# eridgd/WCT-TF

Hardware: AMD Instinct MI355X
Metric: stylized frames/sec @512x512, 5-level relu5->1 pipeline, alpha=0.8 (higher is better)
Workload: dtype f16

## Files before the change

wct_tf_amd/csrc/common.h:

```cpp
#pragma once
#include <hip/hip_runtime.h>
#include <stdint.h>
#include <stddef.h>
#include "skip_rule.h"

typedef _Float16 half_t;
typedef _Float16 half8 __attribute__((ext_vector_type(8)));
typedef _Float16 half4 __attribute__((ext_vector_type(4)));
typedef float f32x16 __attribute__((ext_vector_type(16)));
typedef float f32x4 __attribute__((ext_vector_type(4)));

#define WCT_OK 0
#define WCT_ERR_HIP -1
#define WCT_ERR_ARG -2
#define WCT_ERR_STATE -3
#define WCT_ERR_NOMEM -4
#define WCT_ERR_NOCONV -5

void wct_set_error(const char* fmt, ...);

#define HIP_TRY(expr)                                                          \
  do {                                                                         \
    hipError_t _e = (expr);                                                    \
    if (_e != hipSuccess) {                                                    \
      wct_set_error("%s failed: %s (%s:%d)", #expr, hipGetErrorString(_e),     \
                    __FILE__, __LINE__);                                       \
      return WCT_ERR_HIP;                                                      \
    }                                                                          \
  } while (0)

#define ARG_CHECK(cond)                                                        \
  do {                                                                         \
    if (!(cond)) {                                                             \
      wct_set_error("invalid argument: %s (%s:%d)", #cond, __FILE__, __LINE__);\
      return WCT_ERR_ARG;                                                      \
    }                                                                          \
  } while (0)

static inline int cdiv(int a, int b) { return (a + b - 1) / b; }

constexpr size_t WCT_LAUNCH_BYTES = (size_t)1 << 31;
static inline bool launch_map_fits(size_t elems, size_t bytes) { return elems * bytes < WCT_LAUNCH_BYTES; }


struct ConvArgs {
  const half_t* x;
  const half_t* w;
  const float* bias;
  half_t* y16;
  float* y32;
  int B, H, W;
  int Cin, Cout;
  int upsample;
  int relu;
  int pool;
  float* usum;
  unsigned* umax;
  const float* img1 = nullptr;
  const half_t* w1frag = nullptr;
  const float* bias1 = nullptr;
  int clamp01 = 0;
  const half_t* w_wino = nullptr;
};
constexpr int UMAX_SLOTS = 64;
__device__ __forceinline__ void umax_merge(unsigned* umax_img, int slot, float vmax, int lane) {
#pragma unroll
  for (int o = 32; o > 0; o >>= 1) vmax = fmaxf(vmax, __shfl_xor(vmax, o, 64));
  if (lane == 0) {
    unsigned* w = umax_img + (slot & (UMAX_SLOTS - 1));
    const unsigned bits = __builtin_bit_cast(unsigned, vmax);
    if (bits > __atomic_load_n(w, __ATOMIC_RELAXED)) atomicMax(w, bits);
  }
}
int launch_conv3x3(const ConvArgs& a, hipStream_t s);
bool conv3x3_wino_takes(const ConvArgs& a);
int launch_conv3x3_wino(const ConvArgs& a, hipStream_t s);

struct ConvFirstArgs {
  const float* x;
  const half_t* wfrag;
  const float* bias;
  half_t* y16;
  float* y32;
  int B, H, W;
  int clamp01;
  float* usum;
  unsigned* umax;
};

__device__ __forceinline__ void unit_row_sum4(f32x4& t) {
  float a = t[0], b = t[1], c = t[2], d = t[3];
#define WCT_DPP_STEP(ctrl)                                                             \
  "v_add_f32_dpp %0, %0, %0 " ctrl " row_mask:0xf bank_mask:0xf bound_ctrl:1\n"       \
  "v_add_f32_dpp %1, %1, %1 " ctrl " row_mask:0xf bank_mask:0xf bound_ctrl:1\n"       \
  "v_add_f32_dpp %2, %2, %2 " ctrl " row_mask:0xf bank_mask:0xf bound_ctrl:1\n"       \
  "v_add_f32_dpp %3, %3, %3 " ctrl " row_mask:0xf bank_mask:0xf bound_ctrl:1\n"
  asm volatile("s_nop 1\n"
               WCT_DPP_STEP("quad_perm:[1,0,3,2]")
               WCT_DPP_STEP("quad_perm:[2,3,0,1]")
               WCT_DPP_STEP("row_half_mirror")
               WCT_DPP_STEP("row_mirror")
               : "+v"(a), "+v"(b), "+v"(c), "+v"(d));
#undef WCT_DPP_STEP
  t[0] = a; t[1] = b; t[2] = c; t[3] = d;
}
int launch_conv_first(const ConvFirstArgs& a, hipStream_t s);

struct ConvLastArgs {
  const half_t* x;
  const half_t* wfrag;
  const float* bias;
  float* y;
  int B, H, W;
};
int launch_conv_last(const ConvLastArgs& a, hipStream_t s);

int launch_maxpool2x2(const half_t* x, half_t* y, int B, int H, int W, int C, hipStream_t s);
int launch_u8_to_f32(const uint8_t* x, float* y, size_t n, hipStream_t s);
int launch_f32_to_u8(const float* x, uint8_t* y, size_t n, hipStream_t s);
int launch_f32_to_f16(const float* x, half_t* y, size_t n, hipStream_t s);
int launch_f16_to_f32(const half_t* x, float* y, size_t n, hipStream_t s);

struct GemmArgs {
  const float* A; int lda; int a_kmajor;
  const float* B; int ldb; int b_kmajor;
  const float* a_sub_m;
  const float* b_sub_n;
  const float* a_sub_k;
  const float* a_scale_k;
  int M, N, K;
  int ksplit;
  float* out32; half_t* out16; int ldo;
  size_t out_split_stride;
  const float* bias_n;
  int nsplit;
  size_t sA, sB, s_sub_m, s_sub_n, s_sub_k, s_scale_k, s_out, s_bias;
  const float* A_odd;
  size_t sA_odd;
  WctSkip skip;
  int blend; float alpha; unsigned* mabs;
  const float* mask_diag; size_t s_mask; int* mask_out; const int* mask_in;
};

int launch_gemm(GemmArgs g, int nsplit, int nbatch, hipStream_t s);

enum { WCT_MODE_NP = 0, WCT_MODE_TF = 1 };

struct WctFeatStats { const float* u[2]; const unsigned* umax[2]; };

struct WctImageSide { const float* img; int H, W, clamp01; };
struct WctImageSrc { WctImageSide side[2]; const half_t* wfrag; const float* bias; };

struct WctStyleKey { int nslab, nsplit, ksplit; };
WctStyleKey wct_style_key(int C, int Nc, int Ns);
size_t wct_style_state_floats(int C);
size_t wct_style_workspace_bytes(int C, int Ns, const WctStyleKey& key);
struct WctStyleRef { const float* state[8]; };
struct WctStyleSlots { const float* state[32]; };

struct WctWarmRef { float* basis; int valid; };

struct WctStrength { const uint8_t* smap; int Hm, Wm, w, stride; };

struct WctCall {
  float alpha; int mode;
  float eps;
  half_t* out16; float* out32;
  void* workspace; size_t workspace_bytes;
  int* sweeps_dev;
  int stages;
  int* eig_fail;
  hipStream_t stream;
};
enum { WCT_STAGE_COV = 1, WCT_STAGE_EIG = 2, WCT_STAGE_APPLY = 4, WCT_STAGE_ALL = 7, WCT_STAGE_EIG_FP32UPDATE = 8 };

int launch_style_state(const float* style, int Ns, int C, const WctStyleKey& key, int adain, const WctCall& r, float* state);

size_t wct_workspace_bytes(int C, int Nc, int Ns, int P);
int launch_wct(const float* content, int Nc, const float* style, int Ns, int C, int P, WctSkip skip, const WctCall& r,
               const WctFeatStats* stats, const WctStyleRef* prep, const WctWarmRef* warm, const WctStrength* sm = nullptr,
               const WctImageSrc* src = nullptr );
int launch_adain(const float* content, int Nc, const float* style, int Ns, int C, int P, WctSkip skip, const WctCall& r,
                 const WctFeatStats* stats, const WctStyleRef* prep, const WctStrength* sm = nullptr);
enum { WCT_MIX_MAX = 8 };
size_t wct_mix_workspace_bytes(int C, int Nc, const int* Ns, int K, const float* lambda);
int launch_wct_mix(const float* content, int Nc, const float* const* styles, const int* Ns, int K, const float* lambda, int C,
                   const WctCall& r, const WctFeatStats* stats, const WctStyleRef* prep);
int launch_adain_mix(const float* content, int Nc, const float* const* styles, const int* Ns, int K, const float* lambda, int C,
                     const WctCall& r, const WctFeatStats* stats, const WctStyleRef* prep);
struct MaskGeom { const uint8_t* mask; int Hm, Wm, w, stride; };
size_t mask_compact_workspace_bytes(int N, int G = 1);
int launch_mask_compact(const MaskGeom& g, int N, int K, int* perm, int* seg_off, void* workspace, hipStream_t s);
int launch_mask_gather_segment(const float* x, const int* perm, const int* seg_off, int k, int nk, int C, float* xg, hipStream_t s);
size_t wct_masked_workspace_bytes(int C, int Nc, const int* nk, const int* Ns, int K);
int launch_wct_masked(const float* content, int Nc, const MaskGeom& g, const int* nk, const float* const* styles, const int* Ns, int K,
                      int C, const WctCall& r);
int launch_adain_masked(const float* content, int Nc, const MaskGeom& g, const int* nk, const float* const* styles, const int* Ns, int K,
                        int C, const WctCall& r);
size_t wct_masked_batch_workspace_bytes(int C, int Nc, int G, const int* nk, const int* Ns, int K);
int wct_masked_batch_pairs(int G, const int* nk, int K);
int launch_mask_compact_batch(const MaskGeom& g, int N, int K, int G, int* perm, int* seg_off, void* workspace, hipStream_t s);
int launch_wct_masked_batch(const float* content, int Nc, int G, const MaskGeom& g, const int* nk, const int* Ns, int K, int C,
                            const WctCall& r, const WctStyleSlots& states);
int launch_adain_masked_batch(const float* content, int Nc, int G, const MaskGeom& g, const int* nk, const int* Ns, int K, int C,
                              const WctCall& r, const WctStyleSlots& states);
int launch_jacobi_eigh(float* A, float* V, int C, int nmat, void* workspace,
                       size_t workspace_bytes, int* sweeps_done_dev, int* eig_fail, hipStream_t s);
size_t jacobi_workspace_bytes(int C, int nmat);

size_t style_swap_workspace_bytes(int C, int hc, int wc, int hs, int ws, int patch, int stride);
int launch_style_swap(const float* content, int hc, int wc, const float* style, int hs, int ws, int C,
                      float alpha, int patch, int stride, float eps, half_t* out16, float* out32,
                      void* workspace, size_t workspace_bytes, hipStream_t s, int* eig_fail);

int launch_im2col_act(const half_t* x, float* col, int B, int H, int W, int C, int upsample, hipStream_t s);
int launch_im2col_grad(const float* g, float* col, int B, int H, int W, int C, hipStream_t s);
int launch_reflect_fold(const float* gp, float* g, int B, int H, int W, int C, hipStream_t s);
int launch_relu_mask16(float* g, const half_t* act, size_t n, hipStream_t s);
int launch_relu_mask32(float* g, const float* act, size_t n, hipStream_t s);
int launch_upsample_adjoint(const float* gb, float* gs, int B, int h, int w, int C, hipStream_t s);
int launch_maxpool_adjoint(const half_t* pre, const float* gpool, float* gpre, int B, int H, int W, int C, hipStream_t s);
int launch_mse(const float* a, const float* b, size_t n, float weight, float* grad, int accumulate, double* partial,
               float* loss_out, hipStream_t s);
int launch_tv(const float* x, int B, int H, int W, int C, float weight, float* grad, double* partial, float* loss_out, hipStream_t s);
int launch_bias_grad(const float* g, size_t rows, int C, float* partial, float* out, hipStream_t s);
int launch_reduce_slabs(const float* partial, size_t n, int nslab, float* out, hipStream_t s);
int launch_adam(float* w, float* m, float* v, const float* g, size_t n, float lr_t, float b1, float b2, float eps, hipStream_t s);
int launch_pack_conv_frag(const float* w, half_t* frag, int cin, int cout, hipStream_t s);
int launch_pack_conv_wino_frag(const float* w, half_t* frag, int cin, int cout, hipStream_t s);
int launch_pack_last_frag(const float* w, half_t* frag, hipStream_t s);
int launch_transpose_w(const float* w, float* wt, int cin, int cout, int cout_pad, hipStream_t s);
int launch_pad3to4(const float* x, float* y, size_t n, hipStream_t s);
int launch_conv_dgrad(const float* g, const float* wt, int B, int H, int W, int cin, int cout,
                      float* col, float* gp, float* gin, void* scratch, hipStream_t s);
int launch_conv_wgrad(const half_t* x16, int upsample, const float* g, int ldg, int B, int H, int W, int cin, int cout,
                      float* col, float* partial, int nsplit, float* dw, void* scratch, hipStream_t s);
int conv_wgrad_splits(int B, int H, int W);
int launch_pow2_scale(const float* x, size_t n, void* scratch, hipStream_t s);
int launch_conv_first_dgrad(const float* g, const float* wf, float* gp, int B, int H, int W, hipStream_t s);

struct CoralApplyArgs {
  double M[9], src_mean[3], src_std[3], tgt_mean[3], tgt_std[3];
};
int launch_coral_stats(const uint8_t* img, size_t npix, unsigned long long* partial, int nblocks,
                       unsigned long long* out9, hipStream_t s);
int launch_coral_apply(const uint8_t* src, size_t npix, const CoralApplyArgs& a, uint8_t* out_u8,
                       double* out_f64, hipStream_t s);

int launch_content_colors_f32(const float* frame, const void* content, int content_f32, int B, int Ho, int Wo, int Hc, int Wc,
                              uint8_t* out, hipStream_t s);
int launch_content_colors_u8(const uint8_t* stylized, const uint8_t* content, int B, int Ho, int Wo, int Hc, int Wc, uint8_t* out,
                             hipStream_t s);
int launch_content_colors_u8_any(const uint8_t* stylized, const void* content, int content_f32, int B, int Ho, int Wo, int Hc, int Wc,
                                 uint8_t* out, hipStream_t s);

constexpr int GUIDE_GREY = 0, GUIDE_COLOR = 1;
int guided_check(int B, int Ho, int Wo, int Hc, int Wc, int radius, int eps_q, int guide);
size_t guided_workspace_bytes(int B, int Ho, int Wo, int guide);
int launch_guided_filter(const uint8_t* stylized, const void* content, int content_f32, int B, int Ho, int Wo, int Hc, int Wc, int radius,
                         int eps_q, int guide, void* workspace, uint8_t* out, hipStream_t s);
int launch_guided_color(const uint8_t* stylized, const void* content, int content_f32, int B, int Ho, int Wo, int Hc, int Wc, int radius,
                        int eps_q, void* workspace, uint8_t* out, hipStream_t s);
int guided_time_check(int F, int Ho, int Wo, int Hc, int Wc, int radius, int eps_q, int frames_t, int f0, int f1);
int guided_time_max_radius(int frames_t);
int launch_guided_time(const uint8_t* stylized, const void* content, int content_f32, int F, int Ho, int Wo, int Hc, int Wc, int radius,
                       int eps_q, int frames_t, int f0, int f1, void* workspace, uint8_t* out, hipStream_t s);
int guided_motion_check(int F, int Ho, int Wo, int Hc, int Wc, int radius, int eps_q, int frames_t, int f0, int f1, const int32_t* pos);
int launch_guided_motion(const uint8_t* stylized, const uint8_t* content, int F, int Ho, int Wo, int Hc, int Wc, int radius, int eps_q,
                         int frames_t, const int32_t* pos, int f0, int f1, void* workspace, uint8_t* out, hipStream_t s);
int motion_check(int F, int Hc, int Wc, int range);
size_t motion_workspace_bytes(int F, int Hc, int Wc, int range);
int launch_motion_global(const uint8_t* content, int F, int Hc, int Wc, int range, void* workspace, const int32_t** steps, hipStream_t s);

int launch_texture_noise(uint8_t* out, int B, int H, int W, unsigned seed, unsigned first_sample, int smooth, hipStream_t s);

int launch_wrap_pad(const void* in, void* out, int B, int H, int W, int E, int elem_bytes, int t, int b, int l, int r, hipStream_t s);
int launch_wrap_crop(const void* in, void* out, int B, int Hp, int Wp, int E, int elem_bytes, int t, int l, int h, int w, hipStream_t s);

struct ResizeGeom { int H, W, h, w, ksx, ksy, th; };
int resize_check_bytes(int B, int H, int W, int h, int w);
size_t resize_table_ints(int H, int W, int h, int w);
int resize_plan(int H, int W, int h, int w, ResizeGeom* g, int* tabs);
int launch_resize(const uint8_t* in, uint8_t* out, int B, const ResizeGeom& g, const int* tabs_dev, hipStream_t s);
```

wct_tf_amd/csrc/spectral.hip:

```cpp
#include "wct_stages.h"

__device__ __forceinline__ bool pair_resolved(float dp, float dq, float e) { return e * e <= 0.25f * dp * dq; }

constexpr float SPECTRAL_NOISE_CUT = 2.f;
__device__ __forceinline__ float spectral_cut(const float* Am, int C, int tid, float* red) {
  float mn = 0.f;
  for (int i = tid; i < C; i += 256) mn = fminf(mn, Am[(size_t)i * C + i]);
  for (int o = 32; o > 0; o >>= 1) mn = fminf(mn, __shfl_xor(mn, o, 64));
  if ((tid & 63) == 0) red[tid >> 6] = mn;
  __syncthreads();
  mn = fminf(fminf(red[0], red[1]), fminf(red[2], red[3]));
  return fmaxf(1e-5f, -SPECTRAL_NOISE_CUT * mn);
}

__device__ __forceinline__ float spectral_entry(float dp, float dq, float e, bool diag, int kind, float shift, float cut) {
  const bool kp = dp > cut, kq = dq > cut;
  if (diag) return kp ? (kind == 0 ? 1.f / sqrtf(dp + shift) : sqrtf(dp + shift)) : 0.f;
  if (!kp && !kq) return 0.f;
  if (kp && kq) {
    if (!pair_resolved(dp, dq, e)) return 0.f;
    const float sa = sqrtf(dp + shift), sb = sqrtf(dq + shift);
    return kind == 0 ? -e / (sa * sb * (sa + sb)) : e / (sa + sb);
  }
  const float dk = kp ? dp : dq, dd = kp ? dq : dp;
  const float fk = kind == 0 ? 1.f / sqrtf(dk + shift) : sqrtf(dk + shift);
  return e * fk / fmaxf(dk - dd, 2.f * fabsf(e));
}

struct SpectralTile {
  float dp[64], dq[64];
  float mt[64][65];
};
__attribute__((used)) __device__ __forceinline__ void spectral_tile_load(SpectralTile& t, const float* Am, int C, int p0, int q0, int tid) {
  if (tid < 64) t.dp[tid] = p0 + tid < C ? Am[(size_t)(p0 + tid) * C + p0 + tid] : 0.f;
  else if (tid < 128) t.dq[tid - 64] = q0 + tid - 64 < C ? Am[(size_t)(q0 + tid - 64) * C + q0 + tid - 64] : 0.f;
  const int ty = tid >> 4, tx = tid & 15;
#pragma unroll
  for (int i = 0; i < 4; ++i) {
    const int r = q0 + ty * 4 + i, c = p0 + tx * 4;
    f32x4 v = {0.f, 0.f, 0.f, 0.f};
    if (r < C && c < C) v = *reinterpret_cast<const f32x4*>(Am + (size_t)r * C + c);
#pragma unroll
    for (int j = 0; j < 4; ++j) t.mt[ty * 4 + i][tx * 4 + j] = v[j];
  }
}

struct SpecAllArgs {
  const float* A;
  float* G;
  float *N, *R, *Pm;
  const float *X1, *X2;
  int C; float shift; int correct, second; WctSkip skip;
  unsigned* mabs; const float* mean; float* bias; float alpha; int mode;
};

__global__ __launch_bounds__(256) void spectral_open_all_kernel(SpecAllArgs a) {
  __shared__ SpectralTile t;
  const int m = blockIdx.z, p0 = blockIdx.y * 64, q0 = blockIdx.x * 64, tid = threadIdx.x;
  const int C = a.C, kind = m & 1, pair = m >> 1;
  const size_t cc = (size_t)C * C;
  if (kind == 0 && blockIdx.x == 0 && blockIdx.y == 0) {
    if (tid == 0) a.mabs[pair] = 0u;
    const float* mp = a.mean + (size_t)(one_content(a.skip) ? 0 : pair) * 2 * C;
    const float* ms = a.mean + (size_t)(one_style(a.skip) ? 0 : pair) * 2 * C + C;
    for (int i = tid; i < C; i += 256) {
      float b = a.alpha * ms[i];
      if (a.mode == WCT_MODE_TF) b += (1.f - a.alpha) * mp[i];
      a.bias[pair * C + i] = b;
    }
  }
  if (skip_style_mat(m, a.skip)) return;
  __shared__ float cutred[4];
  const float* Am = a.A + m * cc;
  const float cut = spectral_cut(Am, C, tid, cutred);
  spectral_tile_load(t, Am, C, p0, q0, tid);
  __syncthreads();
  const int ty = tid >> 4, tx = tid & 15;
#pragma unroll
  for (int i = 0; i < 4; ++i) {
    const int pl = ty * 4 + i, p = p0 + pl, q = q0 + tx * 4;
    if (p >= C || q >= C) continue;
    const f32x4 av = *reinterpret_cast<const f32x4*>(Am + (size_t)p * C + q);
    const float dp = t.dp[pl];
    f32x4 g, n4 = {0.f, 0.f, 0.f, 0.f}, r4 = n4, p4 = n4;
#pragma unroll
    for (int j = 0; j < 4; ++j) {
      const float dk = t.dq[tx * 4 + j];
      const float em = 0.5f * (av[j] + t.mt[tx * 4 + j][pl]);
      g[j] = spectral_entry(dp, dk, a.correct ? em : 0.f, p == q + j, kind, a.shift, cut);
      if (a.second && p != q + j && dp > cut && dk > cut && pair_resolved(dp, dk, em)) {
        const float sp = sqrtf(dp + a.shift), sk = sqrtf(dk + a.shift);
        n4[j] = em / (sp + sk);
        r4[j] = em / sk;
        p4[j] = n4[j] / sk;
      }
    }
    const size_t o = (size_t)p * C + q;
    *reinterpret_cast<f32x4*>(a.G + m * cc + o) = g;
    if (a.second) {
      *reinterpret_cast<f32x4*>(a.N + m * cc + o) = n4;
      if (kind == 0) { *reinterpret_cast<f32x4*>(a.R + pair * cc + o) = r4; *reinterpret_cast<f32x4*>(a.Pm + pair * cc + o) = p4; }
    }
  }
}

__global__ __launch_bounds__(256) void spectral_add2_all_kernel(SpecAllArgs a) {
  __shared__ float dps[64], dqs[64];
  __shared__ float x1t[64][65], x2t[64][65];
  const int m = blockIdx.z, p0 = blockIdx.y * 64, q0 = blockIdx.x * 64, tid = threadIdx.x;
  if (skip_style_mat(m, a.skip)) return;
  const int C = a.C, kind = m & 1;
  const size_t cc = (size_t)C * C;
  const float* Am = a.A + m * cc;
  float* Gm = a.G + m * cc;
  const float* X2 = a.X2 + m * cc;
  const float* X1 = a.X1 + (size_t)(m >> 1) * cc;
  int near = 0;
  for (int i = tid; i < C; i += 256) {
    const float d = fabsf(Am[(size_t)i * C + i]);
    near |= (d > 3.3e-6f) & (d < 3e-5f);
  }
  if (__syncthreads_or(near)) return;
  __shared__ float cutred[4];
  const float cut = spectral_cut(Am, C, tid, cutred);
  if (tid < 64) dps[tid] = p0 + tid < C ? Am[(size_t)(p0 + tid) * C + p0 + tid] : 0.f;
  else if (tid < 128) dqs[tid - 64] = q0 + tid - 64 < C ? Am[(size_t)(q0 + tid - 64) * C + q0 + tid - 64] : 0.f;
  const int ty = tid >> 4, tx = tid & 15;
#pragma unroll
  for (int i = 0; i < 4; ++i) {
    const int r = q0 + ty * 4 + i, c = p0 + tx * 4;
    f32x4 v1 = {0.f, 0.f, 0.f, 0.f}, v2 = v1;
    if (r < C && c < C) {
      v2 = *reinterpret_cast<const f32x4*>(X2 + (size_t)r * C + c);
      if (kind == 0) v1 = *reinterpret_cast<const f32x4*>(X1 + (size_t)r * C + c);
    }
#pragma unroll
    for (int j = 0; j < 4; ++j) { x2t[ty * 4 + i][tx * 4 + j] = v2[j]; x1t[ty * 4 + i][tx * 4 + j] = v1[j]; }
  }
  __syncthreads();
#pragma unroll
  for (int i = 0; i < 4; ++i) {
    const int pl = ty * 4 + i, p = p0 + pl, q = q0 + tx * 4;
    if (p >= C || q >= C) continue;
    const size_t o = (size_t)p * C + q;
    const f32x4 x2 = *reinterpret_cast<const f32x4*>(X2 + o);
    f32x4 x1 = {0.f, 0.f, 0.f, 0.f};
    if (kind == 0) x1 = *reinterpret_cast<const f32x4*>(X1 + o);
    f32x4 g = *reinterpret_cast<const f32x4*>(Gm + o);
    const float dp = dps[pl];
#pragma unroll
    for (int j = 0; j < 4; ++j) {
      const float dq = dqs[tx * 4 + j];
      if (!(dp > cut && dq > cut)) continue;
      const float sp = sqrtf(dp + a.shift), sq = sqrtf(dq + a.shift);
      float l2;
      if (kind == 1) l2 = -0.5f * (x2[j] + x2t[tx * 4 + j][pl]) / (sp + sq);
      else l2 = (0.5f * (x1[j] + x1t[tx * 4 + j][pl]) + 0.25f * (sp + sq) * (x2[j] + x2t[tx * 4 + j][pl])) / (sp * sq * (sp + sq));
      g[j] += l2;
    }
    *reinterpret_cast<f32x4*>(Gm + o) = g;
  }
}

static GemmArgs level_product(int C, WctSkip skip) {
  GemmArgs g = {};
  g.lda = g.ldb = g.ldo = C; g.M = g.N = g.K = g.ksplit = C; g.sA = g.sB = g.s_out = (size_t)C * C; g.skip = skip;
  return g;
}

static int launch_refresh(const WctCarve& w, int C, int P, WctSkip skip, hipStream_t s) {
  int rc;
  GemmArgs r1 = level_product(C, skip);
  r1.A = w.A0; r1.a_kmajor = 0; r1.B = w.V; r1.b_kmajor = 1; r1.out32 = w.X;
  r1.mask_diag = w.A; r1.s_mask = (size_t)C * C; r1.mask_out = w.refresh;
  if ((rc = launch_gemm(r1, 1, 2 * P, s))) return rc;
  GemmArgs r2 = level_product(C, skip);
  r2.A = w.V; r2.a_kmajor = 1; r2.B = w.X; r2.b_kmajor = 1; r2.out32 = w.A; r2.mask_in = w.refresh;
  return launch_gemm(r2, 1, 2 * P, s);
}

int launch_spectral_tail_refreshed(const WctCarve& w, int C, int P, float alpha, int mode, float eps_in, WctSkip skip, int nwhite,
                                   hipStream_t s) {
  int rc;
  const size_t cc = (size_t)C * C;
  const float shift = mode == WCT_MODE_NP ? (eps_in >= 0.f ? eps_in : 1e-5f) : 0.f;
  const int second = EIG_CORRECT >= 2;
  const dim3 tiles(cdiv(C, 64), cdiv(C, 64), 2 * P);
  SpecAllArgs sa = {};
  sa.A = w.A; sa.G = w.G; sa.C = C; sa.shift = shift; sa.correct = EIG_CORRECT; sa.second = second; sa.skip = skip;
  sa.N = w.S2; float* X2 = sa.N + 2 * P * cc; sa.R = X2 + 2 * P * cc; sa.Pm = sa.R + P * cc; float* X1 = sa.Pm + P * cc;
  sa.X1 = X1; sa.X2 = X2;
  sa.mabs = w.mabs; sa.mean = w.mean; sa.bias = w.bias; sa.alpha = alpha; sa.mode = mode;
  hipLaunchKernelGGL(spectral_open_all_kernel, tiles, dim3(256), 0, s, sa);
  HIP_TRY(hipGetLastError());
  if (second) {
    GemmArgs a = level_product(C, skip);
    a.A = sa.Pm; a.A_odd = sa.N + cc; a.sA_odd = 2 * cc; a.a_kmajor = 0; a.B = sa.N; a.b_kmajor = 1; a.out32 = X2;
    if ((rc = launch_gemm(a, 1, 2 * P, s))) return rc;
    GemmArgs b = level_product(C, WCT_SKIP_NONE);
    b.A = sa.R; b.a_kmajor = 0; b.B = sa.N; b.b_kmajor = 1; b.sB = 2 * cc; b.out32 = X1;
    if (nwhite > 0 && (rc = launch_gemm(b, 1, nwhite, s))) return rc;
    hipLaunchKernelGGL(spectral_add2_all_kernel, tiles, dim3(256), 0, s, sa);
    HIP_TRY(hipGetLastError());
  }
  GemmArgs g = level_product(C, skip);
  g.A = w.V; g.a_kmajor = 0; g.B = w.G; g.b_kmajor = 1; g.out32 = w.X;
  if ((rc = launch_gemm(g, 1, 2 * P, s))) return rc;
  GemmArgs h = level_product(C, skip);
  h.A = w.X; h.a_kmajor = 0; h.B = w.V; h.b_kmajor = 0; h.out32 = w.Tw;
  return launch_gemm(h, 1, 2 * P, s);
}

int launch_spectral_tail(const WctCarve& w, int C, int P, float alpha, int mode, float eps_in, WctSkip skip, int nwhite,
                         hipStream_t s) {
  const int rc = launch_refresh(w, C, P, skip, s);
  return rc ? rc : launch_spectral_tail_refreshed(w, C, P, alpha, mode, eps_in, skip, nwhite, s);
}
```

wct_tf_amd/csrc/stats_gemm.hip:

```cpp
#include "wct_stages.h"
#include "conv_first_tile.h"
#include <type_traits>


struct StatArgs {
  const float* x[2];
  int n[2];
  const float* u[2];
  const unsigned* umax[2];
  const float* mean;
  float* partial;
  float* absmax;
  int C, nslab;
  WctSkip skip;
};

__global__ __launch_bounds__(256) void colsum_kernel(StatArgs p) {
  __shared__ f32x4 red[256];
  const int mat = blockIdx.y, slab = blockIdx.x;
  if (skip_style_mat(mat, p.skip)) return;
  const int b = mat & 1, pair = mat >> 1;
  const int C = p.C, cq = C / 4;
  const int nrp = 256 / cq;
  const int tid = threadIdx.x;
  const int rp = tid / cq, c4 = tid % cq;
  const int N = p.n[b];
  const float* x = p.x[b] + (size_t)pair * N * C;
  f32x4 acc = {0.f, 0.f, 0.f, 0.f};
  float amax = 0.f;
  if (p.mean) {
    const int rows_per_slab = (N + p.nslab - 1) / p.nslab;
    const int r0 = slab * rows_per_slab;
    const int r1 = min(N, r0 + rows_per_slab);
    const f32x4 m = *reinterpret_cast<const f32x4*>(p.mean + mat * C + c4 * 4);
    if (rp < nrp)
      for (int r = r0 + rp; r < r1; r += nrp) {
        f32x4 v = *reinterpret_cast<const f32x4*>(x + (size_t)r * C + c4 * 4);
        v -= m; acc += v * v;
      }
  } else {
    const int units = (N + 15) >> 4;
    const int ups = (units + p.nslab - 1) / p.nslab;
    const int u0 = slab * ups, u1 = min(units, u0 + ups);
    const float* U = p.u[b] ? p.u[b] + (size_t)pair * units * C : nullptr;
    if (rp < nrp)
      for (int u = u0 + rp; u < u1; u += nrp) {
        if (U) {
          acc += *reinterpret_cast<const f32x4*>(U + (size_t)u * C + c4 * 4);
        } else {
          f32x4 t[16];
#pragma unroll
          for (int i = 0; i < 16; ++i) {
            const int r = u * 16 + i;
            t[i] = *reinterpret_cast<const f32x4*>(x + (size_t)min(r, N - 1) * C + c4 * 4);
            if (r >= N) t[i] = f32x4{0.f, 0.f, 0.f, 0.f};
            amax = fmaxf(fmaxf(amax, fmaxf(fabsf(t[i][0]), fabsf(t[i][1]))), fmaxf(fabsf(t[i][2]), fabsf(t[i][3])));
          }
#pragma unroll
          for (int w = 1; w < 16; w <<= 1)
#pragma unroll
            for (int i = 0; i < 16; i += 2 * w) t[i] += t[i + w];
          acc += t[0];
        }
      }
    if (U) amax = __builtin_bit_cast(float, p.umax[b][pair * UMAX_SLOTS + (tid & (UMAX_SLOTS - 1))]);
  }
  red[tid] = acc;
  __syncthreads();
  if (rp == 0) {
    for (int j = 1; j < nrp; ++j) acc += red[j * cq + c4];
    *reinterpret_cast<f32x4*>(p.partial + ((size_t)mat * p.nslab + slab) * C + c4 * 4) = acc;
  }
  if (p.absmax) {
    __syncthreads();
    float* redf = reinterpret_cast<float*>(red);
    redf[tid] = amax;
    __syncthreads();
    for (int st = 128; st > 0; st >>= 1) {
      if (tid < st) redf[tid] = fmaxf(redf[tid], redf[tid + st]);
      __syncthreads();
    }
    if (tid == 0) p.absmax[(size_t)mat * p.nslab + slab] = redf[0];
  }
}

__global__ void colsum_finish_kernel(const float* partial, float* out, int C, int nslab, float d0, float d1, int skip,
                                     const float* absmax = nullptr, float* scale = nullptr) {
  const int mat = blockIdx.y;
  if (skip_style_mat(mat, skip)) return;
  if (scale && blockIdx.x == 0 && threadIdx.x < 64) {
    float m = 0.f;
    for (int i = threadIdx.x; i < nslab; i += 64) m = fmaxf(m, absmax[(size_t)mat * nslab + i]);
    for (int o = 32; o > 0; o >>= 1) m = fmaxf(m, __shfl_xor(m, o, 64));
    if (threadIdx.x == 0) {
      float sc = 1.f;
      if (m > 0.f && m < 1e30f) {
        int e;
        frexpf(2.f * m, &e);
        sc = ldexpf(1.f, 14 - e);
      }
      scale[mat] = sc;
    }
  }
  const int c = blockIdx.x * blockDim.x + threadIdx.x;
  if (c >= C) return;
  float a[8] = {0.f, 0.f, 0.f, 0.f, 0.f, 0.f, 0.f, 0.f};
  const float* pp = partial + (size_t)mat * nslab * C + c;
  int i = 0;
  for (; i + 8 <= nslab; i += 8) {
#pragma unroll
    for (int j = 0; j < 8; ++j) a[j] += pp[(size_t)(i + j) * C];
  }
  for (; i < nslab; ++i) a[i & 7] += pp[(size_t)i * C];
  const float s = ((a[0] + a[1]) + (a[2] + a[3])) + ((a[4] + a[5]) + (a[6] + a[7]));
  out[mat * C + c] = s / ((mat & 1) == 0 ? d0 : d1);
}

constexpr int GK = 16;

template <int BX>
struct GemmStage {
  static constexpr int NV = GK * BX / 4 / 256;
  f32x4 v[NV];
  __device__ __forceinline__ void load(const float* src, int ld, bool kmajor, int k0, int kend, int x0, int X,
                                       const float* sub_x, const float* sub_k, const float* scale_k, int tid) {
#pragma unroll
    for (int i = 0; i < NV; ++i) {
      const int item = tid + i * 256;
      f32x4 t = {0.f, 0.f, 0.f, 0.f};
      if (kmajor) {
        const int k = item / (BX / 4), x4 = item % (BX / 4);
        const int gk = k0 + k, gx = x0 + x4 * 4;
        if (gk < kend && gx < X) {
          t = *reinterpret_cast<const f32x4*>(src + (size_t)gk * ld + gx);
          if (sub_x) t -= *reinterpret_cast<const f32x4*>(sub_x + gx);
        }
      } else {
        const int x = item / (GK / 4), k4 = item % (GK / 4);
        const int gx = x0 + x, gk = k0 + k4 * 4;
        if (gx < X && gk < kend) {
          t = *reinterpret_cast<const f32x4*>(src + (size_t)gx * ld + gk);
          if (sub_k) t -= *reinterpret_cast<const f32x4*>(sub_k + gk);
          if (scale_k) t *= *reinterpret_cast<const f32x4*>(scale_k + gk);
        }
      }
      v[i] = t;
    }
  }
  __device__ __forceinline__ void store(float* lds , bool kmajor, int tid) const {
    constexpr int P = BX + 4;
#pragma unroll
    for (int i = 0; i < NV; ++i) {
      const int item = tid + i * 256;
      if (kmajor) {
        const int k = item / (BX / 4), x4 = item % (BX / 4);
        *reinterpret_cast<f32x4*>(lds + k * P + x4 * 4) = v[i];
      } else {
        const int x = item / (GK / 4), k4 = item % (GK / 4);
#pragma unroll
        for (int j = 0; j < 4; ++j) lds[(k4 * 4 + j) * P + x] = v[i][j];
      }
    }
  }
};

constexpr float REFRESH_RATIO = 1e-4f;
__device__ __forceinline__ bool refresh_needed(const float* Am, int C, int tid) {
  float dmax = 0.f, dmin = 3.0e38f;
  for (int i = tid; i < C; i += 256) {
    const float d = Am[(size_t)i * C + i];
    dmax = fmaxf(dmax, fabsf(d));
    if (d > 3.3e-6f) dmin = fminf(dmin, d);
  }
  for (int o = 32; o > 0; o >>= 1) { dmax = fmaxf(dmax, __shfl_xor(dmax, o, 64)); dmin = fminf(dmin, __shfl_xor(dmin, o, 64)); }
  __shared__ float red[2][4];
  if ((tid & 63) == 0) { red[0][tid >> 6] = dmax; red[1][tid >> 6] = dmin; }
  __syncthreads();
  dmax = fmaxf(fmaxf(red[0][0], red[0][1]), fmaxf(red[0][2], red[0][3]));
  dmin = fminf(fminf(red[1][0], red[1][1]), fminf(red[1][2], red[1][3]));
  return dmin < 3.0e38f && dmin < REFRESH_RATIO * dmax;
}

template <int BM, int BN>
__global__ __launch_bounds__(256, 4) void gemm_f32_kernel(GemmArgs p) {
  constexpr int TM = BM / 64, TN = BN / 64;
  constexpr int PA = BM + 4, PB = BN + 4;
  __shared__ __attribute__((aligned(16))) float As[GK * PA];
  __shared__ __attribute__((aligned(16))) float Bs[GK * PB];
  const int tid = threadIdx.x, lane = tid & 63, wave = tid >> 6;
  const int wm = wave >> 1, wn = wave & 1;
  const int m0 = blockIdx.y * BM, n0 = blockIdx.x * BN;
  const int batch = blockIdx.z / p.nsplit, split = blockIdx.z % p.nsplit;
  if (p.skip != WCT_SKIP_NONE && skip_style_mat(batch, p.skip)) return;
  if (p.mask_in && !p.mask_in[batch]) return;
  if (p.mask_diag) {
    const bool need = refresh_needed(p.mask_diag + batch * p.s_mask, p.M, tid);
    if (p.mask_out && blockIdx.x == 0 && blockIdx.y == 0 && split == 0 && tid == 0) p.mask_out[batch] = need ? 1 : 0;
    if (!need) return;
  }
  const int kbeg = split * p.ksplit;
  const int kend = min(p.K, kbeg + p.ksplit);
  if (p.A_odd) p.A = (batch & 1) ? p.A_odd + (batch >> 1) * p.sA_odd : p.A + (batch >> 1) * p.sA;
  else p.A += batch * p.sA;
  p.B += batch * p.sB;
  if (p.a_sub_m) p.a_sub_m += batch * p.s_sub_m;
  if (p.b_sub_n) p.b_sub_n += batch * p.s_sub_n;
  if (p.a_sub_k) p.a_sub_k += batch * p.s_sub_k;
  if (p.a_scale_k) p.a_scale_k += batch * p.s_scale_k;
  if (p.bias_n) p.bias_n += batch * p.s_bias;

  f32x16 acc[TM][TN];
#pragma unroll
  for (int i = 0; i < TM; ++i)
#pragma unroll
    for (int j = 0; j < TN; ++j)
#pragma unroll
      for (int r = 0; r < 16; ++r) acc[i][j][r] = 0.f;

  GemmStage<BM> sa;
  GemmStage<BN> sb;
  if (kbeg < kend) {
    sa.load(p.A, p.lda, p.a_kmajor, kbeg, kend, m0, p.M, p.a_sub_m, p.a_sub_k, p.a_scale_k, tid);
    sb.load(p.B, p.ldb, p.b_kmajor, kbeg, kend, n0, p.N, p.b_sub_n, nullptr, nullptr, tid);
  }
  for (int k0 = kbeg; k0 < kend; k0 += GK) {
    sa.store(As, p.a_kmajor, tid);
    sb.store(Bs, p.b_kmajor, tid);
    __syncthreads();
    if (k0 + GK < kend) {
      sa.load(p.A, p.lda, p.a_kmajor, k0 + GK, kend, m0, p.M, p.a_sub_m, p.a_sub_k, p.a_scale_k, tid);
      sb.load(p.B, p.ldb, p.b_kmajor, k0 + GK, kend, n0, p.N, p.b_sub_n, nullptr, nullptr, tid);
    }
#pragma unroll
    for (int kk = 0; kk < GK; kk += 2) {
      float a[TM], b[TN];
      const int kr = kk + (lane >> 5);
#pragma unroll
      for (int i = 0; i < TM; ++i) a[i] = As[kr * PA + (wm * TM + i) * 32 + (lane & 31)];
#pragma unroll
      for (int j = 0; j < TN; ++j) b[j] = Bs[kr * PB + (wn * TN + j) * 32 + (lane & 31)];
#pragma unroll
      for (int i = 0; i < TM; ++i)
#pragma unroll
        for (int j = 0; j < TN; ++j)
          acc[i][j] = __builtin_amdgcn_mfma_f32_32x32x2f32(a[i], b[j], acc[i][j], 0, 0, 0);
    }
    __syncthreads();
  }

  float* o32 = p.out32 ? p.out32 + batch * p.s_out + (size_t)split * p.out_split_stride : nullptr;
  half_t* o16 = p.out16 ? p.out16 + batch * p.s_out : nullptr;
  float biasv[TN];
#pragma unroll
  for (int j = 0; j < TN; ++j) {
    const int gn = n0 + (wn * TN + j) * 32 + (lane & 31);
    biasv[j] = (p.bias_n && gn < p.N) ? p.bias_n[gn] : 0.f;
  }
#pragma unroll
  for (int j = 0; j < TN; ++j) asm volatile("" : "+v"(biasv[j]));
  float av = 0.f;
#pragma unroll
  for (int i = 0; i < TM; ++i)
#pragma unroll
    for (int j = 0; j < TN; ++j) {
      const int gn = n0 + (wn * TN + j) * 32 + (lane & 31);
      const float bias = biasv[j];
#pragma unroll
      for (int r = 0; r < 16; ++r) {
        const int gm = m0 + (wm * TM + i) * 32 + (r & 3) + 8 * (r >> 2) + 4 * (lane >> 5);
        if (gm < p.M && gn < p.N) {
          float v = acc[i][j][r] + bias;
          if (p.blend) {
            v = p.alpha * acc[i][j][r];
            if (gm == gn) v += 1.f - p.alpha;
            av = fmaxf(av, fabsf(v));
          }
          if (o32) o32[(size_t)gm * p.ldo + gn] = v;
          if (o16) o16[(size_t)gm * p.ldo + gn] = (half_t)v;
        }
      }
    }
  if (p.blend) {
    for (int o = 32; o > 0; o >>= 1) av = fmaxf(av, __shfl_xor(av, o, 64));
    if (lane == 0 && av < 1e30f) atomicMax(p.mabs + batch, __float_as_uint(av));
  }
}

int launch_gemm(GemmArgs g, int nsplit, int nbatch, hipStream_t s) {
  g.nsplit = nsplit;
  const int gz = nsplit * nbatch;
  const bool small_grid = (long)cdiv(g.M, 128) * cdiv(g.N, 128) * gz < 256;
  if (g.M >= 128 && g.N >= 128 && !small_grid) {
    dim3 grid(cdiv(g.N, 128), cdiv(g.M, 128), gz);
    hipLaunchKernelGGL((gemm_f32_kernel<128, 128>), grid, dim3(256), 0, s, g);
  } else if (g.M >= 128 && !small_grid) {
    dim3 grid(cdiv(g.N, 64), cdiv(g.M, 128), gz);
    hipLaunchKernelGGL((gemm_f32_kernel<128, 64>), grid, dim3(256), 0, s, g);
  } else {
    dim3 grid(cdiv(g.N, 64), cdiv(g.M, 64), gz);
    hipLaunchKernelGGL((gemm_f32_kernel<64, 64>), grid, dim3(256), 0, s, g);
  }
  HIP_TRY(hipGetLastError());
  return WCT_OK;
}

struct CovArgs {
  const float* x[2];
  int n[2];
  const float* mean;
  const float* scale;
  float* partial;
  int C, ksplit, nsplit, ntile;
  WctSkip skip;
};

template <int BT>
__global__ __launch_bounds__(256, 2) void cov_f16x2_kernel(CovArgs p) {
  constexpr int TM = BT / 64;
  constexpr int KPT = BT * 32 / 256;
  constexpr int NPC = KPT / 8;
  __shared__ __attribute__((aligned(16))) unsigned char lds[4][BT * 64];
  const int tid = threadIdx.x, lane = tid & 63, wave = tid >> 6;
  const int wm = wave >> 1, wn = wave & 1;
  int ti = 0, rem = blockIdx.x;
  while (rem >= p.ntile - ti) { rem -= p.ntile - ti; ++ti; }
  const int tj = ti + rem;
  const bool diag = ti == tj;
  const int m0 = ti * BT, n0 = tj * BT;
  const int mat = blockIdx.z, split = blockIdx.y;
  if (skip_style_mat(mat, p.skip)) return;
  const int side = mat & 1, pair = mat >> 1;
  const int N = p.n[side], C = p.C;
  const float* x = p.x[side] + (size_t)pair * N * C;
  const int kbeg = split * p.ksplit;
  const int kend = min(N, kbeg + p.ksplit);
  const float sc = p.scale[mat];

  const int c = tid % BT;
  const int kg = __builtin_amdgcn_readfirstlane(tid / BT);
  const float mean_a = p.mean[mat * C + min(m0 + c, C - 1)];
  const float mean_b = p.mean[mat * C + min(n0 + c, C - 1)];
  const __amdgpu_buffer_rsrc_t rsrc = __builtin_amdgcn_make_buffer_rsrc((void*)x, 0, (int)((size_t)N * C * 4), 0x00020000);
  const int voff_a = min(m0 + c, C - 1) * 4, voff_b = min(n0 + c, C - 1) * 4;

  f32x16 acc[TM][TM];
#pragma unroll
  for (int i = 0; i < TM; ++i)
#pragma unroll
    for (int j = 0; j < TM; ++j)
#pragma unroll
      for (int r = 0; r < 16; ++r) acc[i][j][r] = 0.f;

  auto load = [&](float (&r)[KPT], int voff, int k0) {
#pragma unroll
    for (int j = 0; j < KPT; ++j)
      r[j] = __builtin_bit_cast(float, __builtin_amdgcn_raw_buffer_load_b32(rsrc, voff, (k0 + kg * KPT + j) * C * 4, 0));
  };
  auto split_store = [&](const float (&r)[KPT], float mean, int k0, bool tail, unsigned char* hi, unsigned char* lo) {
#pragma unroll
    for (int q = 0; q < NPC; ++q) {
      half8 h, l;
#pragma unroll
      for (int j = 0; j < 8; ++j) {
        const float s_in = (!tail || k0 + kg * KPT + q * 8 + j < kend) ? sc : 0.f;
        const float v = (r[q * 8 + j] - mean) * s_in;
        h[j] = (half_t)v;
        l[j] = (half_t)(v - (float)h[j]);
      }
      const int chunk = kg * NPC + q;
      const int off = (c * 4 + (chunk ^ ((c >> 2) & 3))) * 16;
      *reinterpret_cast<half8*>(hi + off) = h;
      *reinterpret_cast<half8*>(lo + off) = l;
    }
  };
  auto mma_stage = [&](const unsigned char* bh, const unsigned char* bl) {
#pragma unroll
    for (int ks = 0; ks < 2; ++ks) {
      const int chunk = ks * 2 + (lane >> 5);
      half8 ah[TM], al[TM], bhf[TM], blf[TM];
#pragma unroll
      for (int i = 0; i < TM; ++i) {
        const int r = (wm * TM + i) * 32 + (lane & 31);
        const int off = (r * 4 + (chunk ^ ((r >> 2) & 3))) * 16;
        ah[i] = *reinterpret_cast<const half8*>(lds[0] + off);
        al[i] = *reinterpret_cast<const half8*>(lds[1] + off);
      }
#pragma unroll
      for (int j = 0; j < TM; ++j) {
        const int r = (wn * TM + j) * 32 + (lane & 31);
        const int off = (r * 4 + (chunk ^ ((r >> 2) & 3))) * 16;
        bhf[j] = *reinterpret_cast<const half8*>(bh + off);
        blf[j] = *reinterpret_cast<const half8*>(bl + off);
      }
#pragma unroll
      for (int i = 0; i < TM; ++i)
#pragma unroll
        for (int j = 0; j < TM; ++j) {
          acc[i][j] = __builtin_amdgcn_mfma_f32_32x32x16_f16(al[i], bhf[j], acc[i][j], 0, 0, 0);
          acc[i][j] = __builtin_amdgcn_mfma_f32_32x32x16_f16(ah[i], blf[j], acc[i][j], 0, 0, 0);
          acc[i][j] = __builtin_amdgcn_mfma_f32_32x32x16_f16(ah[i], bhf[j], acc[i][j], 0, 0, 0);
        }
    }
  };

  float ra[KPT], rb[KPT];
  if (diag) {
    if (kbeg < kend) load(ra, voff_a, kbeg);
    for (int k0 = kbeg; k0 < kend; k0 += 32) {
      if (k0 + 32 <= kend) split_store(ra, mean_a, k0, false, lds[0], lds[1]);
      else split_store(ra, mean_a, k0, true, lds[0], lds[1]);
      __syncthreads();
      if (k0 + 32 < kend) load(ra, voff_a, k0 + 32);
      mma_stage(lds[0], lds[1]);
      __syncthreads();
    }
  } else {
    if (kbeg < kend) { load(ra, voff_a, kbeg); load(rb, voff_b, kbeg); }
    for (int k0 = kbeg; k0 < kend; k0 += 32) {
      if (k0 + 32 <= kend) {
        split_store(ra, mean_a, k0, false, lds[0], lds[1]);
        split_store(rb, mean_b, k0, false, lds[2], lds[3]);
      } else {
        split_store(ra, mean_a, k0, true, lds[0], lds[1]);
        split_store(rb, mean_b, k0, true, lds[2], lds[3]);
      }
      __syncthreads();
      if (k0 + 32 < kend) { load(ra, voff_a, k0 + 32); load(rb, voff_b, k0 + 32); }
      mma_stage(lds[2], lds[3]);
      __syncthreads();
    }
  }

  float* out = p.partial + ((size_t)mat * p.nsplit + split) * C * C;
#pragma unroll
  for (int i = 0; i < TM; ++i)
#pragma unroll
    for (int j = 0; j < TM; ++j) {
      const int gn = n0 + (wn * TM + j) * 32 + (lane & 31);
#pragma unroll
      for (int r = 0; r < 16; ++r) {
        const int gm = m0 + (wm * TM + i) * 32 + (r & 3) + 8 * (r >> 2) + 4 * (lane >> 5);
        if (gm < C && gn < C) out[(size_t)gm * C + gn] = acc[i][j][r];
      }
    }
}

__global__ __launch_bounds__(256) void cov_finish_kernel(const float* partial, const float* scale, float* cov, int C, int nsplit, int BT,
                                                         float inv0, float inv1, float eps, int skip, float* cov0 = nullptr) {
  __shared__ float tt[64][65];
  const int mat = blockIdx.z;
  if (skip_style_mat(mat, skip)) return;
  const size_t cc = (size_t)C * C;
  const int r0 = blockIdx.y * 64, c0 = blockIdx.x * 64, tid = threadIdx.x, ty = tid >> 4, tx = tid & 15;
  const bool mirror = r0 / BT > c0 / BT;
  const float* pb = partial + (size_t)mat * nsplit * cc;
  const float sc = scale[mat];
  const float f = ((mat & 1) == 0 ? inv0 : inv1) / (sc * sc);
  f32x4 acc[4];
#pragma unroll
  for (int i = 0; i < 4; ++i) {
    const int r = (mirror ? c0 : r0) + ty * 4 + i, c = (mirror ? r0 : c0) + tx * 4;
    f32x4 sum = {0.f, 0.f, 0.f, 0.f};
    if (r < C && c < C)
      for (int k = 0; k < nsplit; ++k) sum += *reinterpret_cast<const f32x4*>(pb + (size_t)k * cc + (size_t)r * C + c);
    acc[i] = sum;
  }
  if (mirror) {
#pragma unroll
    for (int i = 0; i < 4; ++i)
#pragma unroll
      for (int j = 0; j < 4; ++j) tt[ty * 4 + i][tx * 4 + j] = acc[i][j];
    __syncthreads();
#pragma unroll
    for (int i = 0; i < 4; ++i)
#pragma unroll
      for (int j = 0; j < 4; ++j) acc[i][j] = tt[tx * 4 + j][ty * 4 + i];
  }
#pragma unroll
  for (int i = 0; i < 4; ++i) {
    const int r = r0 + ty * 4 + i, c = c0 + tx * 4;
    if (r >= C || c >= C) continue;
    f32x4 v = acc[i] * f;
#pragma unroll
    for (int j = 0; j < 4; ++j) if (r == c + j) v[j] += eps;
    *reinterpret_cast<f32x4*>(cov + (size_t)mat * cc + (size_t)r * C + c) = v;
    if (cov0) *reinterpret_cast<f32x4*>(cov0 + (size_t)mat * cc + (size_t)r * C + c) = v;
  }
}

struct CovImageArgs {
  WctImageSrc src;
  const float* mean;
  const float* scale;
  float* partial;
  int ksplit, nsplit;
  WctSkip skip;
};

__global__ __launch_bounds__(256, 2) void cov_image_kernel(CovImageArgs p) {
  constexpr int C = 64;
  __shared__ __attribute__((aligned(16))) unsigned char lds[4][2][C * 64];
  const int tid = threadIdx.x, lane = tid & 63, wave = tid >> 6;
  const int wm = wave >> 1, wn = wave & 1;
  const int mat = blockIdx.z, split = blockIdx.y;
  if (skip_style_mat(mat, p.skip)) return;
  const int side = mat & 1, pair = mat >> 1;
  const int H = side ? p.src.side[1].H : p.src.side[0].H, W = side ? p.src.side[1].W : p.src.side[0].W;
  const int clamp01 = side ? p.src.side[1].clamp01 : p.src.side[0].clamp01;
  const int N = H * W;
  const float* x = (side ? p.src.side[1].img : p.src.side[0].img) + (size_t)pair * N * 3;
  const int kbeg = split * p.ksplit;
  const int kend = min(N, kbeg + p.ksplit);
  const float sc = p.scale[mat];
  const int kgrp = lane >> 5, ch = lane & 31;

  half8 wh[2][2], wl[2][2];
  conv1_weights(p.src.wfrag, lane, wh, wl);
  float bias[2], mean[2];
#pragma unroll
  for (int nt = 0; nt < 2; ++nt) { bias[nt] = p.src.bias[nt * 32 + ch]; mean[nt] = p.mean[mat * C + nt * 32 + ch]; }

  f32x16 acc;
#pragma unroll
  for (int r = 0; r < 16; ++r) acc[r] = 0.f;

  float pre[2][8];
  int py, px;
  {
    const int n = kbeg + wave * 32 + (lane & 31);
    py = n / W; px = n - py * W;
  }
  auto fetch = [&]() {
    conv1_patch_load(x, min(py, H - 1), px, H, W, kgrp, pre);
    px += 128;
    while (px >= W) { px -= W; ++py; }
  };
  auto mma_stage = [&](const unsigned char* hi, const unsigned char* lo) {
#pragma unroll
    for (int ks = 0; ks < 2; ++ks) {
      const int chunk = ks * 2 + (lane >> 5);
      const int ra = wm * 32 + (lane & 31), rb = wn * 32 + (lane & 31);
      const int offa = (ra * 4 + (chunk ^ ((ra >> 2) & 3))) * 16, offb = (rb * 4 + (chunk ^ ((rb >> 2) & 3))) * 16;
      const half8 ah = *reinterpret_cast<const half8*>(hi + offa), al = *reinterpret_cast<const half8*>(lo + offa);
      const half8 bh = *reinterpret_cast<const half8*>(hi + offb), bl = *reinterpret_cast<const half8*>(lo + offb);
      acc = __builtin_amdgcn_mfma_f32_32x32x16_f16(al, bh, acc, 0, 0, 0);
      acc = __builtin_amdgcn_mfma_f32_32x32x16_f16(ah, bl, acc, 0, 0, 0);
      acc = __builtin_amdgcn_mfma_f32_32x32x16_f16(ah, bh, acc, 0, 0, 0);
    }
  };

  auto park = [&](const f32x16 (&f)[2], int ks0, auto tail) {
#pragma unroll
    for (int nt = 0; nt < 2; ++nt) {
      const int c = nt * 32 + ch;
#pragma unroll
      for (int rq = 0; rq < 4; ++rq) {
        half4 h, l;
#pragma unroll
        for (int j = 0; j < 4; ++j) {
          const float s_in = (!decltype(tail)::value || ks0 + rq * 8 + kgrp * 4 + j < kend) ? sc : 0.f;
          const float v = (conv1_act(f[nt][rq * 4 + j], bias[nt]) - mean[nt]) * s_in;
          h[j] = (half_t)v;
          l[j] = (half_t)(v - (float)h[j]);
        }
        const int off = (c * 4 + (rq ^ ((c >> 2) & 3))) * 16 + kgrp * 8;
        *reinterpret_cast<half4*>(lds[wave][0] + off) = h;
        *reinterpret_cast<half4*>(lds[wave][1] + off) = l;
      }
    }
  };

  if (kbeg + wave * 32 < kend) fetch();
  for (int k0 = kbeg; k0 < kend; k0 += 128) {
    const int ks0 = k0 + wave * 32;
    if (ks0 < kend) {
      float cur[2][8];
      conv1_patch_values(pre, kgrp, clamp01, cur);
      if (ks0 + 128 < kend) fetch();
      f32x16 f[2];
      conv1_tile<true>(wh, wl, [=](int ks, int j) { return cur[ks][j]; }, f);
      if (ks0 + 32 <= kend) park(f, ks0, std::false_type());
      else park(f, ks0, std::true_type());
    }
    __syncthreads();
#pragma unroll
    for (int st = 0; st < 4; ++st)
      if (k0 + st * 32 < kend) mma_stage(lds[st][0], lds[st][1]);
    __syncthreads();
  }

  float* out = p.partial + ((size_t)mat * p.nsplit + split) * C * C;
  const int gn = wn * 32 + (lane & 31);
#pragma unroll
  for (int r = 0; r < 16; ++r) {
    const int gm = wm * 32 + (r & 3) + 8 * (r >> 2) + 4 * (lane >> 5);
// ... 98 lines not shown
```

Baseline: 676.2.

## Compute only upper-triangle tiles for symmetric GEMM outputs and mirror via transpose

Result: no change. 679.2 (median of 6 runs) (+0.4%).

```diff
diff --git a/wct_tf_amd/csrc/common.h b/wct_tf_amd/csrc/common.h
--- a/wct_tf_amd/csrc/common.h
+++ b/wct_tf_amd/csrc/common.h
@@ -140,6 +140,7 @@
   WctSkip skip;
   int blend; float alpha; unsigned* mabs;
   const float* mask_diag; size_t s_mask; int* mask_out; const int* mask_in;
+  int sym_out;
 };
 
 int launch_gemm(GemmArgs g, int nsplit, int nbatch, hipStream_t s);
diff --git a/wct_tf_amd/csrc/spectral.hip b/wct_tf_amd/csrc/spectral.hip
--- a/wct_tf_amd/csrc/spectral.hip
+++ b/wct_tf_amd/csrc/spectral.hip
@@ -196,6 +196,7 @@
   if (second) {
     GemmArgs a = level_product(C, skip);
     a.A = sa.Pm; a.A_odd = sa.N + cc; a.sA_odd = 2 * cc; a.a_kmajor = 0; a.B = sa.N; a.b_kmajor = 1; a.out32 = X2;
+    a.sym_out = 1;
     if ((rc = launch_gemm(a, 1, 2 * P, s))) return rc;
     GemmArgs b = level_product(C, WCT_SKIP_NONE);
     b.A = sa.R; b.a_kmajor = 0; b.B = sa.N; b.b_kmajor = 1; b.sB = 2 * cc; b.out32 = X1;
@@ -208,6 +209,7 @@
   if ((rc = launch_gemm(g, 1, 2 * P, s))) return rc;
   GemmArgs h = level_product(C, skip);
   h.A = w.X; h.a_kmajor = 0; h.B = w.V; h.b_kmajor = 0; h.out32 = w.Tw;
+  h.sym_out = 1;
   return launch_gemm(h, 1, 2 * P, s);
 }
 
diff --git a/wct_tf_amd/csrc/stats_gemm.hip b/wct_tf_amd/csrc/stats_gemm.hip
--- a/wct_tf_amd/csrc/stats_gemm.hip
+++ b/wct_tf_amd/csrc/stats_gemm.hip
@@ -1,5 +1,6 @@
 #include "wct_stages.h"
 #include "conv_first_tile.h"
+#include "sym_tiles.h"
 #include <type_traits>
 
 
@@ -181,15 +182,28 @@
   return dmin < 3.0e38f && dmin < REFRESH_RATIO * dmax;
 }
 
-template <int BM, int BN>
-__global__ __launch_bounds__(256, 4) void gemm_f32_kernel(GemmArgs p) {
+template <int BM, int BN, bool SYM>
+__device__ __forceinline__ void gemm_f32_tile(GemmArgs p) {
   constexpr int TM = BM / 64, TN = BN / 64;
   constexpr int PA = BM + 4, PB = BN + 4;
-  __shared__ __attribute__((aligned(16))) float As[GK * PA];
-  __shared__ __attribute__((aligned(16))) float Bs[GK * PB];
+  __shared__ __attribute__((aligned(16))) float As[SYM ? 1 : GK * PA];
+  __shared__ __attribute__((aligned(16))) float Bs[SYM ? 1 : GK * PB];
+  constexpr int NSTAGE = GK * (PA + PB), NTURN = 4 * 32 * 33;
+  __shared__ __attribute__((aligned(16))) float Sym[SYM ? (NSTAGE > NTURN ? NSTAGE : NTURN) : 1];
+  float* const as = SYM ? Sym : As;
+  float* const bs = SYM ? Sym + GK * PA : Bs;
   const int tid = threadIdx.x, lane = tid & 63, wave = tid >> 6;
   const int wm = wave >> 1, wn = wave & 1;
-  const int m0 = blockIdx.y * BM, n0 = blockIdx.x * BN;
+  int m0 = blockIdx.y * BM, n0 = blockIdx.x * BN;
+  bool own = true, turn = false, any_turn = false;
+  if constexpr (SYM) {
+    int ti, tj;
+    sym_tile(blockIdx.x, (p.M + BM - 1) / BM, &ti, &tj);
+    m0 = ti * BM; n0 = tj * BN;
+    own = ti != tj || BM == 64 || wm <= wn;
+    turn = ti != tj || (BM == 128 && wm < wn);
+    any_turn = ti != tj || BM == 128;
+  }
   const int batch = blockIdx.z / p.nsplit, split = blockIdx.z % p.nsplit;
   if (p.skip != WCT_SKIP_NONE && skip_style_mat(batch, p.skip)) return;
   if (p.mask_in && !p.mask_in[batch]) return;
@@ -224,8 +238,8 @@
     sb.load(p.B, p.ldb, p.b_kmajor, kbeg, kend, n0, p.N, p.b_sub_n, nullptr, nullptr, tid);
   }
   for (int k0 = kbeg; k0 < kend; k0 += GK) {
-    sa.store(As, p.a_kmajor, tid);
-    sb.store(Bs, p.b_kmajor, tid);
+    sa.store(as, p.a_kmajor, tid);
+    sb.store(bs, p.b_kmajor, tid);
     __syncthreads();
     if (k0 + GK < kend) {
       sa.load(p.A, p.lda, p.a_kmajor, k0 + GK, kend, m0, p.M, p.a_sub_m, p.a_sub_k, p.a_scale_k, tid);
@@ -236,9 +250,9 @@
       float a[TM], b[TN];
       const int kr = kk + (lane >> 5);
 #pragma unroll
-      for (int i = 0; i < TM; ++i) a[i] = As[kr * PA + (wm * TM + i) * 32 + (lane & 31)];
-#pragma unroll
-      for (int j = 0; j < TN; ++j) b[j] = Bs[kr * PB + (wn * TN + j) * 32 + (lane & 31)];
+      for (int i = 0; i < TM; ++i) a[i] = as[kr * PA + (wm * TM + i) * 32 + (lane & 31)];
+#pragma unroll
+      for (int j = 0; j < TN; ++j) b[j] = bs[kr * PB + (wn * TN + j) * 32 + (lane & 31)];
 #pragma unroll
       for (int i = 0; i < TM; ++i)
 #pragma unroll
@@ -268,7 +282,7 @@
 #pragma unroll
       for (int r = 0; r < 16; ++r) {
         const int gm = m0 + (wm * TM + i) * 32 + (r & 3) + 8 * (r >> 2) + 4 * (lane >> 5);
-        if (gm < p.M && gn < p.N) {
+        if (gm < p.M && gn < p.N && (!SYM || own)) {
           float v = acc[i][j][r] + bias;
           if (p.blend) {
             v = p.alpha * acc[i][j][r];
@@ -284,13 +298,57 @@
     for (int o = 32; o > 0; o >>= 1) av = fmaxf(av, __shfl_xor(av, o, 64));
     if (lane == 0 && av < 1e30f) atomicMax(p.mabs + batch, __float_as_uint(av));
   }
+  if constexpr (SYM) {
+    if (!any_turn) return;
+    float* const ts = Sym + wave * (32 * 33);
+#pragma unroll
+    for (int i = 0; i < TM; ++i)
+#pragma unroll
+      for (int j = 0; j < TN; ++j) {
+        __syncthreads();
+        if (turn) {
+#pragma unroll
+          for (int r = 0; r < 16; ++r) ts[((r & 3) + 8 * (r >> 2) + 4 * (lane >> 5)) * 33 + (lane & 31)] = acc[i][j][r] + biasv[j];
+        }
+        __syncthreads();
+        if (!turn) continue;
+        const int gr0 = n0 + (wn * TN + j) * 32, gc0 = m0 + (wm * TM + i) * 32;
+#pragma unroll
+        for (int it = 0; it < 4; ++it) {
+          const int item = lane + it * 64, c = item >> 3, r4 = (item & 7) * 4;
+          if (gr0 + c < p.N && gc0 + r4 < p.M) {
+            const f32x4 t = {ts[r4 * 33 + c], ts[(r4 + 1) * 33 + c], ts[(r4 + 2) * 33 + c], ts[(r4 + 3) * 33 + c]};
+            *reinterpret_cast<f32x4*>(o32 + (size_t)(gr0 + c) * p.ldo + gc0 + r4) = t;
+          }
+        }
+      }
+  }
+}
+
+template <int BM, int BN>
+__global__ __launch_bounds__(256, 4) void gemm_f32_kernel(GemmArgs p) {
+  gemm_f32_tile<BM, BN, false>(p);
+}
+
+template <int BT>
+__global__ __launch_bounds__(256, 4) void gemm_f32_sym_kernel(GemmArgs p) {
+  gemm_f32_tile<BT, BT, true>(p);
 }
 
 int launch_gemm(GemmArgs g, int nsplit, int nbatch, hipStream_t s) {
   g.nsplit = nsplit;
   const int gz = nsplit * nbatch;
   const bool small_grid = (long)cdiv(g.M, 128) * cdiv(g.N, 128) * gz < 256;
-  if (g.M >= 128 && g.N >= 128 && !small_grid) {
+  if (g.sym_out) {
+    ARG_CHECK(g.M == g.N && g.M % 4 == 0 && g.ldo % 4 == 0 && g.out32 && !g.out16 && !g.bias_n && !g.blend && !g.mask_out);
+    if (g.M >= 128 && !small_grid) {
+      dim3 grid(sym_tile_count(cdiv(g.M, 128)), 1, gz);
+      hipLaunchKernelGGL((gemm_f32_sym_kernel<128>), grid, dim3(256), 0, s, g);
+    } else {
+      dim3 grid(sym_tile_count(cdiv(g.M, 64)), 1, gz);
+      hipLaunchKernelGGL((gemm_f32_sym_kernel<64>), grid, dim3(256), 0, s, g);
+    }
+  } else if (g.M >= 128 && g.N >= 128 && !small_grid) {
     dim3 grid(cdiv(g.N, 128), cdiv(g.M, 128), gz);
     hipLaunchKernelGGL((gemm_f32_kernel<128, 128>), grid, dim3(256), 0, s, g);
   } else if (g.M >= 128 && !small_grid) {
diff --git a/wct_tf_amd/csrc/sym_tiles.h b/wct_tf_amd/csrc/sym_tiles.h
--- /dev/null
+++ b/wct_tf_amd/csrc/sym_tiles.h
@@ -0,0 +1,16 @@
+#pragma once
+
+#if defined(__HIPCC__)
+#define WCT_SYM_HD __device__ __host__ __forceinline__
+#else
+#define WCT_SYM_HD inline
+#endif
+
+WCT_SYM_HD int sym_tile_count(int nt) { return nt * (nt + 1) / 2; }
+
+WCT_SYM_HD void sym_tile(int b, int nt, int* ti, int* tj) {
+  int i = 0;
+  while (b >= nt - i) { b -= nt - i; ++i; }
+  *ti = i;
+  *tj = i + b;
+}
```
